# crisbodnar/text-to-image

Measured on AMD Instinct MI355X. Metric: images/sec (G+D step) at 64x64 batch=64, higher is better.
Workload: dtype f32; 1 GPU; wgancls 64x64 batch=64/GPU fp32, synthetic images + random 1024-d text embeddings, D step (+kt) then G step, Adam(b1=0,b2=0.9); global_batch=64, parallelism=dp1, launch=hipGraph replay (1 graph/iteration)

## Files before the change

### text-to-image_amd/csrc/t2i_bgemm.hip

```cpp
#include <hip/hip_runtime.h>
#include <stdint.h>

#include <type_traits>

#include "t2i_internal.h"

namespace t2i {

typedef float f32x16 __attribute__((ext_vector_type(16)));
typedef unsigned int u32x4 __attribute__((ext_vector_type(4)));

namespace {
constexpr int BK = 32;
constexpr int KSTRIDE = BK + 4;
constexpr unsigned OOB = 0xFFFFFFF0u;

template <int LAY, int WM, int WN, int NW = 4>
struct BSmem {
  static constexpr bool A_KIN = LAY != 2, B_KIN = LAY == 1;
  static constexpr int BM = 32 * (NW / 2) * WM, BN = 64 * WN;
  static constexpr int A_ELEMS = A_KIN ? BM * KSTRIDE : BK * BM;
  static constexpr int B_ELEMS = B_KIN ? BN * KSTRIDE : BK * BN;
  static constexpr int BYTES = 2 * (A_ELEMS + B_ELEMS) * 4;
};
// ... 84 lines not shown
        b_ok[i] = n < p.N;
        b_off[i] = (b_kr + B_KR * i) * p.N + n;
      }
    }
  };

  float4 areg[A_LD], breg[B_LD];
  auto load_into = [&](float4* ar, float4* br) __attribute__((always_inline)) {
    const int k0 = l_t * BK;
    ++l_t;
#pragma unroll
    for (int i = 0; i < A_LD; ++i) {
      if (A_KIN) ar[i] = bl4(ra, a_off[i] + k0, a_ok[i] & (k0 + kq * 4 < p.K));
      else ar[i] = bl4(ra, a_off[i] + k0 * p.M, a_ok[i] & (k0 + a_kr + A_KR * i < p.K));
    }
#pragma unroll
    for (int i = 0; i < B_LD; ++i) {
      if (B_KIN) br[i] = bl4(rb, b_off[i] + k0, b_ok[i] & (k0 + kq * 4 < p.K));
      else br[i] = bl4(rb, b_off[i] + k0 * p.N, b_ok[i] & (k0 + b_kr + B_KR * i < p.K));
    }
  };
  auto load_tile = [&]() __attribute__((always_inline)) { load_into(areg, breg); };
  auto store_from = [&](int buf, const float4* ar, const float4* br) __attribute__((always_inline)) {
    float* as = As + buf * S::A_ELEMS;
    float* bs = Bs + buf * S::B_ELEMS;
#pragma unroll
    for (int i = 0; i < A_LD; ++i) {
      if (A_KIN) *reinterpret_cast<float4*>(&as[(r0 + RPP * i) * KSTRIDE + kq * 4]) = ar[i];
      else *reinterpret_cast<float4*>(&as[(a_kr + A_KR * i) * BM + a_c4 * 4]) = ar[i];
    }
#pragma unroll
    for (int i = 0; i < B_LD; ++i) {
      if (B_KIN) *reinterpret_cast<float4*>(&bs[(r0 + RPP * i) * KSTRIDE + kq * 4]) = br[i];
      else *reinterpret_cast<float4*>(&bs[(b_kr + B_KR * i) * BN + b_c4 * 4]) = br[i];
    }
  };
  auto store_tile = [&](int buf) __attribute__((always_inline)) { store_from(buf, areg, breg); };

  struct Frag { float a[WM][4]; float b[WN][4]; };
  auto read_frag = [&](Frag& f, const float* as, const float* bs, int c) __attribute__((always_inline)) {
#pragma unroll
    for (int i = 0; i < WM; ++i) {
      const int row = (wm * WM + i) * 32 + l31;
      if (A_KIN) {
        const float4 v = *reinterpret_cast<const float4*>(&as[row * KSTRIDE + c * 8 + lh * 4]);
        f.a[i][0] = v.x; f.a[i][1] = v.y; f.a[i][2] = v.z; f.a[i][3] = v.w;
      } else {
#pragma unroll
        for (int j = 0; j < 4; ++j) f.a[i][j] = as[(c * 8 + j + 4 * lh) * BM + row];
      }
    }
#pragma unroll
    for (int i = 0; i < WN; ++i) {
      const int col = (wn * WN + i) * 32 + l31;
      if (B_KIN) {
        const float4 v = *reinterpret_cast<const float4*>(&bs[col * KSTRIDE + c * 8 + lh * 4]);
        f.b[i][0] = v.x; f.b[i][1] = v.y; f.b[i][2] = v.z; f.b[i][3] = v.w;
      } else {
#pragma unroll
        for (int j = 0; j < 4; ++j) f.b[i][j] = bs[(c * 8 + j + 4 * lh) * BN + col];
      }
    }
  };

  f32x16 acc[WM][WN];
#pragma unroll
  for (int i = 0; i < WM; ++i)
#pragma unroll
    for (int n = 0; n < WN; ++n)
#pragma unroll
      for (int e = 0; e < 16; ++e) acc[i][n][e] = 0.f;
  auto mma_frag = [&](const Frag& f) __attribute__((always_inline)) {
#pragma unroll
    for (int j = 0; j < 4; ++j)
#pragma unroll
      for (int i = 0; i < WM; ++i)
#pragma unroll
        for (int n = 0; n < WN; ++n)
          acc[i][n] = __builtin_amdgcn_mfma_f32_32x32x2f32(f.a[i][j], f.b[n][j], acc[i][n], 0, 0, 0);
  };
  constexpr int N_MMA = 4 * WM * WN, N_PIECE = A_LD + B_LD, MMA_PER_PIECE = N_MMA / N_PIECE > 0 ? N_MMA / N_PIECE : 1;

  auto k_tile = [&](int t, Frag& c0, Frag& c1, Frag& n0, Frag& n1) __attribute__((always_inline)) {
    const float* as = As + (t & 1) * S::A_ELEMS;
    const float* bs = Bs + (t & 1) * S::B_ELEMS;
    const float* an = As + ((t + 1) & 1) * S::A_ELEMS;
    const float* bn_ = Bs + ((t + 1) & 1) * S::B_ELEMS;
    __builtin_amdgcn_sched_barrier(0);
    mma_frag(c0);
    __builtin_amdgcn_sched_barrier(0);
    read_frag(c0, as, bs, 2);
    __builtin_amdgcn_sched_barrier(0);
    mma_frag(c1);
    store_tile((t + 1) & 1);
#pragma unroll
    for (int q2 = 0; q2 < N_PIECE; ++q2) {
      __builtin_amdgcn_sched_group_barrier(0x008, MMA_PER_PIECE, 0);
      __builtin_amdgcn_sched_group_barrier(0x200, 1, 0);
    }
    __builtin_amdgcn_sched_barrier(0);
    read_frag(c1, as, bs, 3);
    __builtin_amdgcn_sched_barrier(0);
    __syncthreads();
    read_frag(n0, an, bn_, 0);
    read_frag(n1, an, bn_, 1);
    __builtin_amdgcn_sched_barrier(0);
    load_tile();
    mma_frag(c0);
#pragma unroll
    for (int q2 = 0; q2 < N_PIECE; ++q2) {
      __builtin_amdgcn_sched_group_barrier(0x008, MMA_PER_PIECE, 0);
      __builtin_amdgcn_sched_group_barrier(0x020, 1, 0);
    }
    __builtin_amdgcn_sched_barrier(0);
    mma_frag(c1);
  };

  next_item();
  {
    float4 a0[A_LD], b0[B_LD];
    load_into(a0, b0);
    load_tile();
    store_from(0, a0, b0);
  }
  __syncthreads();
  Frag fa0, fa1, fb0, fb1;
  read_frag(fa0, As, Bs, 0);
  read_frag(fa1, As, Bs, 1);
  for (int it = 0; it < n_items; ++it) {
    for (int t = 0; t < p.ntiles; t += 2) {
      if (t + 2 == p.ntiles) next_item();
      k_tile(0, fa0, fa1, fb0, fb1);
      k_tile(1, fb0, fb1, fa0, fa1);
    }
    int bz, bm, bn;
    coords(run0 + slot + it * nslot, bz, bm, bn);
    float* out = p.c + (int64_t)bz * p.sc;
#pragma unroll
    for (int i = 0; i < WM; ++i)
#pragma unroll
      for (int j = 0; j < WN; ++j) {
        const int n = bn + (wn * WN + j) * 32 + l31;
#pragma unroll
        for (int e = 0; e < 16; ++e) {
          const int m = bm + (wm * WM + i) * 32 + (e & 3) + 8 * (e >> 2) + 4 * lh;
          if (m < p.M && n < p.N) out[(size_t)m * p.N + n] = acc[i][j][e];
        }
#pragma unroll
        for (int e = 0; e < 16; ++e) acc[i][j][e] = 0.f;
      }
  }
}

template <int LAY, bool XF = false>
__global__ __launch_bounds__(256, 2) void bgemm9_kernel(Bgemm9Params q) {
  static_assert(!XF, "the in-loader input transform is the specialisation bgemm9_kernel<1, true> below");
  const BgemmParams& p = q.g;
  using S = BSmem<LAY, 1, 1, 4>;
  constexpr bool B_KIN = S::B_KIN;
  constexpr int BM = 64, BN = 64, A_LD = 2, B_LD = 2;
  constexpr int B_C4 = BN / 4, B_KR = 256 / B_C4;
  extern __shared__ __attribute__((aligned(16))) float smem_b[];
  float* As = smem_b;
  float* Bs = smem_b + 2 * S::A_ELEMS;

  const int tid = threadIdx.x;
  const int lane = tid & 63, wave = tid >> 6;
  const int wm = wave >> 1, wn = wave & 1;
  const int l31 = lane & 31, lh = lane >> 5;

  const int nslot = gridDim.x >> 3;
  const int xcd = blockIdx.x & 7, slot = blockIdx.x >> 3;
  const int qq = p.items >> 3, rr_ = p.items & 7;
  const int run0 = xcd * qq + min(xcd, rr_), runlen = qq + (xcd < rr_ ? 1 : 0);
  if (slot >= runlen) return;
  const int n_items = (runlen - slot + nslot - 1) / nslot;
  const int tiles = p.tiles_m * p.tiles_n;

  auto coords = [&](int w, int& phs, int& bm, int& bn) __attribute__((always_inline)) {
    phs = w / tiles;
    const int t = w - phs * tiles;
    const int g = p.group_n, per_group = g * p.tiles_m;
    const int grp = t / per_group, rr = t - grp * per_group, n0 = grp * g;
    const int width = min(g, p.tiles_n - n0);
    const int tm = rr / width;
    bm = tm * BM;
    bn = (n0 + rr - tm * width) * BN;
  };
  auto plane_slot = [&](int pos, int phs) __attribute__((always_inline)) {
    if (LAY == 0) return pos;
    const int r = pos / 3, c = pos - 3 * r;
    return ((2 - r) * 3 + (2 - c)) * 4 + (3 - phs);
  };

  const int kq = tid & 7, r0 = tid >> 3;
  const int b_c4 = tid % B_C4, b_kr = tid / B_C4;
  __amdgpu_buffer_rsrc_t ra, rb;
  int a_off[A_LD], b_off[B_LD];
  bool a_ok[A_LD], b_ok[B_LD];
  int l_item = -1, l_pos = 8, l_t = 0, l_phs = 0, l_bm = 0, l_bn = 0;

  auto next_sub = [&]() __attribute__((always_inline)) {
    l_t = 0;
    if (++l_pos == 9) {
      l_pos = 0;
      ++l_item;
      if (l_item < n_items) coords(run0 + slot + l_item * nslot, l_phs, l_bm, l_bn);
    }
    if (l_item >= n_items) {
#pragma unroll
      for (int i = 0; i < A_LD; ++i) a_ok[i] = false;
#pragma unroll
      for (int i = 0; i < B_LD; ++i) b_ok[i] = false;
      return;
    }
    const int ps = plane_slot(l_pos, l_phs);
    ra = __builtin_amdgcn_make_buffer_rsrc(const_cast<float*>(p.a + (int64_t)ps * p.sa), (short)0, (int)p.a_bytes, 0x00020000);
    rb = __builtin_amdgcn_make_buffer_rsrc(const_cast<float*>(p.b + (int64_t)ps * p.sb), (short)0, (int)p.b_bytes, 0x00020000);
#pragma unroll
    for (int i = 0; i < A_LD; ++i) {
      const int m = l_bm + r0 + 32 * i;
      a_ok[i] = m < p.M;
      a_off[i] = m * p.K + kq * 4;
    }
#pragma unroll
    for (int i = 0; i < B_LD; ++i) {
      if (B_KIN) {
        const int n = l_bn + r0 + 32 * i;
        b_ok[i] = n < p.N;
        b_off[i] = n * p.K + kq * 4;
      } else {
        const int n = l_bn + b_c4 * 4;
        b_ok[i] = n < p.N;
        b_off[i] = (b_kr + B_KR * i) * p.N + n;
      }
    }
  };

  float4 areg[A_LD], breg[B_LD];
  auto load_into = [&](float4* ar, float4* br) __attribute__((always_inline)) {
    const int k0 = l_t * BK;
    ++l_t;
#pragma unroll
    for (int i = 0; i < A_LD; ++i) ar[i] = bl4(ra, a_off[i] + k0, a_ok[i] & (k0 + kq * 4 < p.K));
#pragma unroll
    for (int i = 0; i < B_LD; ++i) {
      if (B_KIN) br[i] = bl4(rb, b_off[i] + k0, b_ok[i] & (k0 + kq * 4 < p.K));
      else br[i] = bl4(rb, b_off[i] + k0 * p.N, b_ok[i] & (k0 + b_kr + B_KR * i < p.K));
    }
  };
  auto store_from = [&](int buf, const float4* ar, const float4* br) __attribute__((always_inline)) {
    float* as = As + buf * S::A_ELEMS;
    float* bs = Bs + buf * S::B_ELEMS;
#pragma unroll
    for (int i = 0; i < A_LD; ++i) *reinterpret_cast<float4*>(&as[(r0 + 32 * i) * KSTRIDE + kq * 4]) = ar[i];
#pragma unroll
    for (int i = 0; i < B_LD; ++i) {
      if (B_KIN) *reinterpret_cast<float4*>(&bs[(r0 + 32 * i) * KSTRIDE + kq * 4]) = br[i];
      else *reinterpret_cast<float4*>(&bs[(b_kr + B_KR * i) * BN + b_c4 * 4]) = br[i];
    }
  };

  struct Frag { float a[4]; float b[4]; };
  auto read_frag = [&](Frag& f, const float* as, const float* bs, int c) __attribute__((always_inline)) {
    {
      const int row = wm * 32 + l31;
      const float4 v = *reinterpret_cast<const float4*>(&as[row * KSTRIDE + c * 8 + lh * 4]);
      f.a[0] = v.x; f.a[1] = v.y; f.a[2] = v.z; f.a[3] = v.w;
    }
    {
      const int col = wn * 32 + l31;
      if (B_KIN) {
        const float4 v = *reinterpret_cast<const float4*>(&bs[col * KSTRIDE + c * 8 + lh * 4]);
        f.b[0] = v.x; f.b[1] = v.y; f.b[2] = v.z; f.b[3] = v.w;
      } else {
#pragma unroll
        for (int j = 0; j < 4; ++j) f.b[j] = bs[(c * 8 + j + 4 * lh) * BN + col];
      }
    }
  };

  f32x16 acc[9];
#pragma unroll
  for (int i = 0; i < 9; ++i)
#pragma unroll
    for (int e = 0; e < 16; ++e) acc[i][e] = 0.f;

  auto k_tile = [&](auto P_, int t, Frag& c0, Frag& c1, Frag& n0, Frag& n1) __attribute__((always_inline)) {
    constexpr int P = decltype(P_)::value;
    const float* as = As + (t & 1) * S::A_ELEMS;
    const float* bs = Bs + (t & 1) * S::B_ELEMS;
    const float* an = As + ((t + 1) & 1) * S::A_ELEMS;
    const float* bn_ = Bs + ((t + 1) & 1) * S::B_ELEMS;
    auto mma = [&](const Frag& f) __attribute__((always_inline)) {
#pragma unroll
      for (int j = 0; j < 4; ++j) acc[P] = __builtin_amdgcn_mfma_f32_32x32x2f32(f.a[j], f.b[j], acc[P], 0, 0, 0);
    };
    __builtin_amdgcn_sched_barrier(0);
    mma(c0);
    __builtin_amdgcn_sched_barrier(0);
    read_frag(c0, as, bs, 2);
    __builtin_amdgcn_sched_barrier(0);
    mma(c1);
    store_from((t + 1) & 1, areg, breg);
#pragma unroll
    for (int q2 = 0; q2 < 4; ++q2) {
      __builtin_amdgcn_sched_group_barrier(0x008, 1, 0);
      __builtin_amdgcn_sched_group_barrier(0x200, 1, 0);
    }
    __builtin_amdgcn_sched_barrier(0);
    read_frag(c1, as, bs, 3);
    __builtin_amdgcn_sched_barrier(0);
    __syncthreads();
    read_frag(n0, an, bn_, 0);
    read_frag(n1, an, bn_, 1);
    __builtin_amdgcn_sched_barrier(0);
    load_into(areg, breg);
    mma(c0);
#pragma unroll
    for (int q2 = 0; q2 < 4; ++q2) {
      __builtin_amdgcn_sched_group_barrier(0x008, 1, 0);
      __builtin_amdgcn_sched_group_barrier(0x020, 1, 0);
    }
    __builtin_amdgcn_sched_barrier(0);
    mma(c1);
  };

  next_sub();
  {
    float4 a0[A_LD], b0[B_LD];
    load_into(a0, b0);
    load_into(areg, breg);
    store_from(0, a0, b0);
  }
  __syncthreads();
  Frag fa0, fa1, fb0, fb1;
  read_frag(fa0, As, Bs, 0);
  read_frag(fa1, As, Bs, 1);
  auto run_pos = [&](auto P_) __attribute__((always_inline)) {
    for (int t = 0; t < p.ntiles; t += 2) {
      if (t + 2 == p.ntiles) next_sub();
      k_tile(P_, 0, fa0, fa1, fb0, fb1);
      k_tile(P_, 1, fb0, fb1, fa0, fa1);
    }
  };
  const int plane_px = q.Th * q.Tw;
  for (int it = 0; it < n_items; ++it) {
    run_pos(std::integral_constant<int, 0>{}); run_pos(std::integral_constant<int, 1>{}); run_pos(std::integral_constant<int, 2>{});
    run_pos(std::integral_constant<int, 3>{}); run_pos(std::integral_constant<int, 4>{}); run_pos(std::integral_constant<int, 5>{});
    run_pos(std::integral_constant<int, 6>{}); run_pos(std::integral_constant<int, 7>{}); run_pos(std::integral_constant<int, 8>{});
    int phs, bm, bn;
    coords(run0 + slot + it * nslot, phs, bm, bn);
    const int ph = phs >> 1, pw = phs & 1;
    const int n = bn + wn * 32 + l31;
    const float bs_ = (q.bias && n < p.N) ? q.bias[n] : 0.f;
#pragma unroll
    for (int e = 0; e < 16; ++e) {
      const int m = bm + wm * 32 + (e & 3) + 8 * (e >> 2) + 4 * lh;
      float z[2][3];
#pragma unroll
      for (int c = 0; c < 3; ++c) {
        z[0][c] = acc[0 * 3 + c][e] + acc[1 * 3 + c][e];
        z[1][c] = acc[1 * 3 + c][e] + acc[2 * 3 + c][e];
      }
      if (m < p.M && n < p.N) {
        const int b = m / plane_px, rem = m - b * plane_px;
        const int ty = rem / q.Tw, tx = rem - ty * q.Tw;
#pragma unroll
        for (int r = 0; r < 2; ++r) {
          const float y0 = apply_act((z[r][0] + z[r][1]) + bs_, q.act, q.alpha);
          const float y1 = apply_act((z[r][1] + z[r][2]) + bs_, q.act, q.alpha);
          const size_t oh = (size_t)q.sr * (2 * ty + r) + ph, ow0 = (size_t)q.sr * (2 * tx) + pw;
          float* o = q.out + (((size_t)b * q.OH + oh) * q.OW + ow0) * p.N + n;
          o[0] = y0;
          o[(size_t)q.sr * p.N] = y1;
        }
      }
    }
#pragma unroll
    for (int i = 0; i < 9; ++i)
#pragma unroll
      for (int e = 0; e < 16; ++e) acc[i][e] = 0.f;
  }
}

namespace {
__host__ __device__ constexpr int w9_pos(int i) {
  return i == 0 ? 4 : i == 1 ? 1 : i == 2 ? 3 : i == 3 ? 0 : i == 4 ? 5 : i == 5 ? 2 : i == 6 ? 7 : i == 7 ? 6 : 8;
}
constexpr int W9_PARK_BYTES = 4 * 2 * 256 * 16;
__device__ __forceinline__ float4 sub4(float4 a, float4 b) { return make_float4(a.x - b.x, a.y - b.y, a.z - b.z, a.w - b.w); }
}

template <>
__global__ __launch_bounds__(256, 2) void bgemm9_kernel<1, true>(Bgemm9Params q) {
  const BgemmParams& p = q.g;
  using S = BSmem<1, 1, 1, 4>;
  constexpr int BM = 64, BN = 64;
  extern __shared__ __attribute__((aligned(16))) float smem_b[];
  float* As = smem_b;
  float* Bs = smem_b + 2 * S::A_ELEMS;

  const int tid = threadIdx.x;
  const int lane = tid & 63, wave = tid >> 6;
  const int wm = wave >> 1, wn = wave & 1;
  const int l31 = lane & 31, lh = lane >> 5;
  float4* park = reinterpret_cast<float4*>(smem_b + 2 * (S::A_ELEMS + S::B_ELEMS)) + tid;

  const int nslot = gridDim.x >> 3;
  const int xcd = blockIdx.x & 7, slot = blockIdx.x >> 3;
  const int qq = p.items >> 3, rr_ = p.items & 7;
  const int run0 = xcd * qq + min(xcd, rr_), runlen = qq + (xcd < rr_ ? 1 : 0);
  if (slot >= runlen) return;
  const int n_items = (runlen - slot + nslot - 1) / nslot;
  const int tiles = p.tiles_m * p.tiles_n;

  auto coords = [&](int w, int& phs, int& bm, int& bn) __attribute__((always_inline)) {
    phs = w / tiles;
    const int t = w - phs * tiles;
    const int g = p.group_n, per_group = g * p.tiles_m;
    const int grp = t / per_group, rr = t - grp * per_group, n0 = grp * g;
    const int width = min(g, p.tiles_n - n0);
    const int tm = rr / width;
    bm = tm * BM;
    bn = (n0 + rr - tm * width) * BN;
  };

  const int kq = tid & 7, r0 = tid >> 3;
  const __amdgpu_buffer_rsrc_t ra = __builtin_amdgcn_make_buffer_rsrc(const_cast<float*>(q.dy), (short)0, (int)p.a_bytes, 0x00020000);
  const int rowpx = q.dWo * p.K;
  int a_off[2], b_off[2];
  unsigned a_win[2];
  bool b_ok[2];
  int l_item = -1, l_t = p.ntiles - 1, l_phs = 0;

  auto advance = [&]() __attribute__((always_inline)) {
    if (++l_t < p.ntiles) return;
    l_t = 0;
    ++l_item;
    if (l_item >= n_items) {
#pragma unroll
      for (int i = 0; i < 2; ++i) { a_win[i] = 0u; b_ok[i] = false; }
      return;
    }
    int bm, bn;
    coords(run0 + slot + l_item * nslot, l_phs, bm, bn);
    const int ph = l_phs >> 1, pw = l_phs & 1;
#pragma unroll
    for (int i = 0; i < 2; ++i) {
      const int m = bm + r0 + 32 * i;
      const int b = m / (q.Th * q.Tw), rem = m - b * (q.Th * q.Tw);
      const int ty = rem / q.Tw, tx = rem - ty * q.Tw;
      const int oh0 = 2 * ty + ph - 1, ow0 = 2 * tx + pw - 1;
      a_off[i] = ((b * q.dHo + oh0) * q.dWo + ow0) * p.K + kq * 4;
      unsigned w = 0u;
#pragma unroll
      for (int rr2 = 0; rr2 < 3; ++rr2)
#pragma unroll
        for (int cc2 = 0; cc2 < 3; ++cc2)
          if ((unsigned)(oh0 + rr2) < (unsigned)q.dHo && (unsigned)(ow0 + cc2) < (unsigned)q.dWo) w |= 1u << (rr2 * 3 + cc2);
      a_win[i] = m < p.M ? w : 0u;
      const int n = bn + r0 + 32 * i;
      b_ok[i] = n < p.N;
      b_off[i] = n * p.K + kq * 4;
    }
  };

  float4 areg[2], breg[2];
  auto load_stage = [&](auto I_, float4* ar, float4* br) __attribute__((always_inline)) {
    constexpr int P = w9_pos(decltype(I_)::value), r = P / 3, c = P - 3 * r;
    const int k0 = l_t * BK;
    const bool kin = k0 + kq * 4 < p.K;
    const int tap = r * rowpx + c * p.K + k0;
#pragma unroll
    for (int i = 0; i < 2; ++i) ar[i] = bl4(ra, a_off[i] + tap, kin & (((a_win[i] >> P) & 1u) != 0u));
    const int ps = ((2 - r) * 3 + (2 - c)) * 4 + (3 - l_phs);
    const __amdgpu_buffer_rsrc_t rb = __builtin_amdgcn_make_buffer_rsrc(const_cast<float*>(p.b + (int64_t)ps * p.sb), (short)0, (int)p.b_bytes, 0x00020000);
#pragma unroll
    for (int i = 0; i < 2; ++i) br[i] = bl4(rb, b_off[i] + k0, b_ok[i] & kin);
  };

  float4 c4[2];
  auto park_read = [&](auto I_, float4* tb, float4* tc) __attribute__((always_inline)) {
    constexpr int P = w9_pos(decltype(I_)::value), r = P / 3, c = P - 3 * r;
    if (r != 1 && c != 1) {
#pragma unroll
      for (int i = 0; i < 2; ++i) {
        tb[i] = park[(((3 + c) - 1) / 2 * 2 + i) * 256];
        tc[i] = park[(((3 * r + 1) - 1) / 2 * 2 + i) * 256];
      }
    }
  };
  auto form_store = [&](auto I_, int buf, const float4* ar, const float4* br, const float4* pb, const float4* pc) __attribute__((always_inline)) {
    constexpr int P = w9_pos(decltype(I_)::value), r = P / 3, c = P - 3 * r;
    float* as = As + buf * S::A_ELEMS;
    float* bs = Bs + buf * S::B_ELEMS;
    const float4 zero = make_float4(0.f, 0.f, 0.f, 0.f);
#pragma unroll
    for (int i = 0; i < 2; ++i) *reinterpret_cast<float4*>(&bs[(r0 + 32 * i) * KSTRIDE + kq * 4]) = br[i];
    if (P == 4) { c4[0] = ar[0]; c4[1] = ar[1]; }
    if ((P & 1) != 0) {
#pragma unroll
      for (int i = 0; i < 2; ++i) park[((P - 1) / 2 * 2 + i) * 256] = ar[i];
    }
#pragma unroll
    for (int i = 0; i < 2; ++i) {
      const float4 tb = r == 1 ? zero : c == 1 ? c4[i] : pb[i];
      const float4 tc = c == 1 ? zero : r == 1 ? c4[i] : pc[i];
      const float4 td = (r != 1 && c != 1) ? c4[i] : zero;
      *reinterpret_cast<float4*>(&as[(r0 + 32 * i) * KSTRIDE + kq * 4]) = sub4(sub4(ar[i], tb), sub4(tc, td));
    }
  };

  struct Frag { float a[4]; float b[4]; };
  auto read_frag = [&](Frag& f, const float* as, const float* bs, int c) __attribute__((always_inline)) {
    const float4 va = *reinterpret_cast<const float4*>(&as[(wm * 32 + l31) * KSTRIDE + c * 8 + lh * 4]);
    f.a[0] = va.x; f.a[1] = va.y; f.a[2] = va.z; f.a[3] = va.w;
    const float4 vb = *reinterpret_cast<const float4*>(&bs[(wn * 32 + l31) * KSTRIDE + c * 8 + lh * 4]);
    f.b[0] = vb.x; f.b[1] = vb.y; f.b[2] = vb.z; f.b[3] = vb.w;
  };

  f32x16 acc[9];
#pragma unroll
  for (int i = 0; i < 9; ++i)
#pragma unroll
    for (int e = 0; e < 16; ++e) acc[i][e] = 0.f;

  auto k_tile = [&](auto I_, int t, Frag& c0, Frag& c1, Frag& n0, Frag& n1) __attribute__((always_inline)) {
    constexpr int I = decltype(I_)::value, P = w9_pos(I);
    using IN = std::integral_constant<int, (I + 1) % 9>;
    using IL = std::integral_constant<int, (I + 2) % 9>;
    const float* as = As + (t & 1) * S::A_ELEMS;
    const float* bs = Bs + (t & 1) * S::B_ELEMS;
    const float* an = As + ((t + 1) & 1) * S::A_ELEMS;
    const float* bn_ = Bs + ((t + 1) & 1) * S::B_ELEMS;
    auto mma = [&](const Frag& f) __attribute__((always_inline)) {
#pragma unroll
      for (int j = 0; j < 4; ++j) acc[P] = __builtin_amdgcn_mfma_f32_32x32x2f32(f.a[j], f.b[j], acc[P], 0, 0, 0);
    };
    float4 pb[2], pc[2];
    __builtin_amdgcn_sched_barrier(0);
    mma(c0);
    __builtin_amdgcn_sched_barrier(0);
    read_frag(c0, as, bs, 2);
    park_read(IN{}, pb, pc);
    __builtin_amdgcn_sched_barrier(0);
    mma(c1);
    form_store(IN{}, (t + 1) & 1, areg, breg, pb, pc);
#pragma unroll
    for (int q2 = 0; q2 < 4; ++q2) {
      __builtin_amdgcn_sched_group_barrier(0x008, 1, 0);
      __builtin_amdgcn_sched_group_barrier(0x002, 6, 0);
      __builtin_amdgcn_sched_group_barrier(0x200, 2, 0);
    }
    __builtin_amdgcn_sched_barrier(0);
    read_frag(c1, as, bs, 3);
    __builtin_amdgcn_sched_barrier(0);
    __syncthreads();
    read_frag(n0, an, bn_, 0);
    read_frag(n1, an, bn_, 1);
    __builtin_amdgcn_sched_barrier(0);
    load_stage(IL{}, areg, breg);
    mma(c0);
#pragma unroll
    for (int q2 = 0; q2 < 4; ++q2) {
      __builtin_amdgcn_sched_group_barrier(0x008, 1, 0);
      __builtin_amdgcn_sched_group_barrier(0x020, 1, 0);
    }
    __builtin_amdgcn_sched_barrier(0);
    mma(c1);
  };

  advance();
  {
    float4 a0[2], b0[2];
    load_stage(std::integral_constant<int, 0>{}, a0, b0);
    load_stage(std::integral_constant<int, 1>{}, areg, breg);
    form_store(std::integral_constant<int, 0>{}, 0, a0, b0, a0, a0);
  }
  __syncthreads();
  Frag fa0, fa1, fb0, fb1;
  read_frag(fa0, As, Bs, 0);
  read_frag(fa1, As, Bs, 1);
#define T2I_W9_STAGE(I, u) \
  if ((((u) + (I)) & 1) == 0) k_tile(std::integral_constant<int, I>{}, 0, fa0, fa1, fb0, fb1); \
  else k_tile(std::integral_constant<int, I>{}, 1, fb0, fb1, fa0, fa1);
#define T2I_W9_KTILE(u) \
  T2I_W9_STAGE(0, u) T2I_W9_STAGE(1, u) T2I_W9_STAGE(2, u) T2I_W9_STAGE(3, u) T2I_W9_STAGE(4, u) T2I_W9_STAGE(5, u) T2I_W9_STAGE(6, u) \
  advance(); \
  T2I_W9_STAGE(7, u) T2I_W9_STAGE(8, u)
  const int plane_px = q.Th * q.Tw;
  for (int it = 0; it < n_items; ++it) {
    for (int t = 0; t < p.ntiles; t += 2) {
      T2I_W9_KTILE(0)
      T2I_W9_KTILE(1)
    }
#undef T2I_W9_KTILE
#undef T2I_W9_STAGE
    int phs, bm, bn;
    coords(run0 + slot + it * nslot, phs, bm, bn);
    const int ph = phs >> 1, pw = phs & 1;
    const int n = bn + wn * 32 + l31;
    const float bs_ = (q.bias && n < p.N) ? q.bias[n] : 0.f;
#pragma unroll
    for (int e = 0; e < 16; ++e) {
      const int m = bm + wm * 32 + (e & 3) + 8 * (e >> 2) + 4 * lh;
      float z[2][3];
#pragma unroll
      for (int c = 0; c < 3; ++c) {
        z[0][c] = acc[0 * 3 + c][e] + acc[1 * 3 + c][e];
        z[1][c] = acc[1 * 3 + c][e] + acc[2 * 3 + c][e];
      }
      if (m < p.M && n < p.N) {
        const int b = m / plane_px, rem = m - b * plane_px;
        const int ty = rem / q.Tw, tx = rem - ty * q.Tw;
#pragma unroll
        for (int r = 0; r < 2; ++r) {
          const float y0 = apply_act((z[r][0] + z[r][1]) + bs_, q.act, q.alpha);
          const float y1 = apply_act((z[r][1] + z[r][2]) + bs_, q.act, q.alpha);
          const size_t oh = (size_t)q.sr * (2 * ty + r) + ph, ow0 = (size_t)q.sr * (2 * tx) + pw;
          float* o = q.out + (((size_t)b * q.OH + oh) * q.OW + ow0) * p.N + n;
          o[0] = y0;
          o[(size_t)q.sr * p.N] = y1;
        }
      }
    }
#pragma unroll
    for (int i = 0; i < 9; ++i)
#pragma unroll
      for (int e = 0; e < 16; ++e) acc[i][e] = 0.f;
  }
}

hipError_t bgemm9_launch(int lay, const Bgemm9Params& q, hipStream_t stream) {
  if (lay != 0 && lay != 1) return hipErrorInvalidValue;
  const int bytes = lay == 0 ? BSmem<0, 1, 1, 4>::BYTES : BSmem<1, 1, 1, 4>::BYTES;
  const int per_xcd = (q.g.items + 7) / 8;
  int nslot = per_xcd < 32 * 2 ? per_xcd : 32 * 2;
  if (nslot < 1) nslot = 1;
  if (lay == 0) hipLaunchKernelGGL((bgemm9_kernel<0, false>), dim3(nslot * 8), dim3(256), bytes, stream, q);
  else if (q.dy) {
    constexpr int wbytes = BSmem<1, 1, 1, 4>::BYTES + W9_PARK_BYTES;
    static bool attr_done = false;
    if (!attr_done) {
      hipError_t e = hipFuncSetAttribute(reinterpret_cast<const void*>(bgemm9_kernel<1, true>), hipFuncAttributeMaxDynamicSharedMemorySize, wbytes);
      if (e != hipSuccess) return e;
      attr_done = true;
    }
    hipLaunchKernelGGL((bgemm9_kernel<1, true>), dim3(nslot * 8), dim3(256), wbytes, stream, q);
  } else hipLaunchKernelGGL((bgemm9_kernel<1, false>), dim3(nslot * 8), dim3(256), bytes, stream, q);
  return hipGetLastError();
}

template <int LAY, int WM, int WN, int NW = 4>
static hipError_t launch_b(const BgemmParams& p, hipStream_t stream) {
  using S = BSmem<LAY, WM, WN, NW>;
  auto k = bgemm_kernel<LAY, WM, WN, NW>;
  static bool attr_done = false;
  if (!attr_done && S::BYTES > 48 * 1024) {
    hipError_t e = hipFuncSetAttribute(reinterpret_cast<const void*>(k), hipFuncAttributeMaxDynamicSharedMemorySize, S::BYTES);
    if (e != hipSuccess) return e;
    attr_done = true;
  }
  const int per_cu = (WM * WN == 1 && NW == 4) ? 4 : 2;
  const int per_xcd = (p.items + 7) / 8;
  int nslot = per_xcd < 32 * per_cu ? per_xcd : 32 * per_cu;
  if (nslot < 1) nslot = 1;
  hipLaunchKernelGGL(k, dim3(nslot * 8), dim3(64 * NW), S::BYTES, stream, p);
  return hipGetLastError();
}

hipError_t bgemm_launch(int lay, int wm, int wn, const BgemmParams& p, hipStream_t stream) {
  if (wm == 4 && wn == 1) {
    if (lay == 0) return launch_b<0, 1, 1, 8>(p, stream);
    if (lay == 1) return launch_b<1, 1, 1, 8>(p, stream);
    if (lay == 2) return launch_b<2, 1, 1, 8>(p, stream);
  }
#define T2I_B(L, a, b) if (lay == L && wm == a && wn == b) return launch_b<L, a, b>(p, stream);
  T2I_B(0, 1, 1) T2I_B(0, 2, 1) T2I_B(0, 1, 2) T2I_B(0, 2, 2)
  T2I_B(1, 1, 1) T2I_B(1, 2, 1) T2I_B(1, 1, 2) T2I_B(1, 2, 2)
  T2I_B(2, 1, 1) T2I_B(2, 2, 1) T2I_B(2, 1, 2) T2I_B(2, 2, 2)
#undef T2I_B
  return hipErrorInvalidValue;
}

}
```

### text-to-image_amd/csrc/t2i_winograd.hip

```cpp
#include <hip/hip_runtime.h>
#include <stdint.h>
#include <stdio.h>
#include <string.h>
#include <stdlib.h>

#include <mutex>
#include <vector>

#include "t2i_internal.h"

namespace t2i {

struct FilterEntry {
  const float* w; int kind, Cin, Cout; float* U; size_t bytes; unsigned long long cap; hipStream_t stream; bool valid;
  hipStream_t cap_fill = nullptr;
};
static std::mutex g_fc_mu;
static std::vector<FilterEntry> g_fc;
static int g_fc_on = 0;
static char* g_fc_buf = nullptr;
static size_t g_fc_cap = 0, g_fc_used = 0;

int filter_cache_attach(void* buf, size_t bytes) {
  std::lock_guard<std::mutex> lk(g_fc_mu);
// ... 342 lines not shown
  const int rc = run_batched_gemm(gd, MODE_BWD_FILTER, 16, V, Z, P, (int64_t)Tp * d.Cin, (int64_t)T * d.Cout, (int64_t)d.Cin * d.Cout, stream,
                                  "winograd filter-gradient gemm");
  if (rc != T2I_OK) return rc;
  hipLaunchKernelGGL(wino_dw_kernel, dim3(wino_blocks((size_t)d.Cin * (d.Cout / 4))), dim3(256), 0, stream, P, d.Cin, d.Cout, accumulate, dw);
  const hipError_t e = hipGetLastError();
  if (e != hipSuccess) { set_error("winograd filter gradient: %s", hipGetErrorString(e)); return T2I_ERR_LAUNCH; }
  return T2I_OK;
}

__device__ __forceinline__ void wino2_filter_body(const float* __restrict__ w, int Cin, int Cout, float* __restrict__ U, unsigned vb, unsigned nvb) {
  const int N4 = Cout >> 2;
  const size_t total = (size_t)4 * Cin * N4;
  const size_t plane = (size_t)4 * Cin * N4;
  for (size_t i = (size_t)vb * 256 + threadIdx.x; i < total; i += (size_t)nvb * 256) {
    const int n4 = (int)(i % N4);
    const int ci = (int)((i / N4) % Cin);
    const int ph = (int)(i / ((size_t)N4 * Cin));
    const int p = ph >> 1, q = ph & 1;
    float4 g[2][2];
#pragma unroll
    for (int a = 0; a < 2; ++a)
#pragma unroll
      for (int b = 0; b < 2; ++b)
        g[a][b] = reinterpret_cast<const float4*>(w + ((size_t)((2 * a + p) * 4 + (2 * b + q)) * Cin + ci) * Cout)[n4];
    float4 s[3][2] = {{g[0][0], g[0][1]}, {f4add(g[0][0], g[1][0]), f4add(g[0][1], g[1][1])}, {g[1][0], g[1][1]}};
    float4* o = reinterpret_cast<float4*>(U) + ((size_t)ph * Cin + ci) * N4 + n4;
#pragma unroll
    for (int r = 0; r < 3; ++r) {
      wst(&o[(size_t)(r * 3 + 0) * plane], s[r][0]);
      wst(&o[(size_t)(r * 3 + 1) * plane], f4add(s[r][0], s[r][1]));
      wst(&o[(size_t)(r * 3 + 2) * plane], s[r][1]);
    }
  }
}

__global__ __launch_bounds__(256) void wino2_filter_kernel(const float* __restrict__ w, int Cin, int Cout, float* __restrict__ U) {
  wino2_filter_body(w, Cin, Cout, U, blockIdx.x, gridDim.x);
}

__global__ __launch_bounds__(256) void wino2_input_kernel(const float* __restrict__ x, int H, int W, int C, int Th, int Tw, size_t T,
                                                          float* __restrict__ V, size_t plane_T) {
  const int C4 = C >> 2;
  const size_t total = T * 4 * C4;
  const size_t plane = plane_T * 4 * C4;
  for (size_t i = (size_t)blockIdx.x * blockDim.x + threadIdx.x; i < total; i += (size_t)gridDim.x * blockDim.x) {
    const int c4 = (int)(i % C4);
    const int ph = (int)((i / C4) & 3);
    const size_t t = i / ((size_t)4 * C4);
    const int p = ph >> 1, q = ph & 1;
    const int tx = (int)(t % Tw);
    const int ty = (int)((t / Tw) % Th);
    const size_t b = t / ((size_t)Tw * Th);
    float4 d[3][3];
#pragma unroll
    for (int r = 0; r < 3; ++r) {
      const int ih = 4 * ty - 1 + 2 * r + p;
#pragma unroll
      for (int c = 0; c < 3; ++c) {
        const int iw = 4 * tx - 1 + 2 * c + q;
        d[r][c] = ((unsigned)ih < (unsigned)H && (unsigned)iw < (unsigned)W)
                      ? reinterpret_cast<const float4*>(x + ((b * H + ih) * W + iw) * C)[c4]
                      : make_float4(0.f, 0.f, 0.f, 0.f);
      }
    }
    float4 tt[3][3];
#pragma unroll
    for (int c = 0; c < 3; ++c) {
      tt[0][c] = f4sub(d[0][c], d[1][c]);
      tt[1][c] = d[1][c];
      tt[2][c] = f4sub(d[2][c], d[1][c]);
    }
    float4* o = reinterpret_cast<float4*>(V) + (t * 4 + ph) * C4 + c4;
#pragma unroll
    for (int r = 0; r < 3; ++r) {
      wst(&o[(size_t)(r * 3 + 0) * plane], f4sub(tt[r][0], tt[r][1]));
      wst(&o[(size_t)(r * 3 + 1) * plane], tt[r][1]);
      wst(&o[(size_t)(r * 3 + 2) * plane], f4sub(tt[r][2], tt[r][1]));
    }
  }
}

__global__ __launch_bounds__(256) void wino2_output_kernel(const float* __restrict__ Mx, const float* __restrict__ bias, int Ho, int Wo,
                                                           int N, int Th, int Tw, size_t T, int act, float alpha,
                                                           float* __restrict__ y) {
  const int N4 = N >> 2;
  const size_t total = T * N4, plane = T * N4;
  for (size_t i = (size_t)blockIdx.x * blockDim.x + threadIdx.x; i < total; i += (size_t)gridDim.x * blockDim.x) {
    const int n4 = (int)(i % N4);
    const size_t t = i / N4;
    const int tx = (int)(t % Tw);
    const int ty = (int)((t / Tw) % Th);
    const size_t b = t / ((size_t)Tw * Th);
    const float4* m = reinterpret_cast<const float4*>(Mx) + t * N4 + n4;
    float4 z[2][3];
#pragma unroll
    for (int c = 0; c < 3; ++c) {
      const float4 m0 = m[(size_t)(0 * 3 + c) * plane], m1 = m[(size_t)(1 * 3 + c) * plane], m2 = m[(size_t)(2 * 3 + c) * plane];
      z[0][c] = f4add(m0, m1);
      z[1][c] = f4add(m1, m2);
    }
    const float4 bs = bias ? reinterpret_cast<const float4*>(bias)[n4] : make_float4(0.f, 0.f, 0.f, 0.f);
#pragma unroll
    for (int r = 0; r < 2; ++r) {
      float4 y0 = f4add(f4add(z[r][0], z[r][1]), bs);
      float4 y1 = f4add(f4add(z[r][1], z[r][2]), bs);
      y0.x = apply_act(y0.x, act, alpha); y0.y = apply_act(y0.y, act, alpha); y0.z = apply_act(y0.z, act, alpha); y0.w = apply_act(y0.w, act, alpha);
      y1.x = apply_act(y1.x, act, alpha); y1.y = apply_act(y1.y, act, alpha); y1.z = apply_act(y1.z, act, alpha); y1.w = apply_act(y1.w, act, alpha);
      float4* o = reinterpret_cast<float4*>(y + ((b * Ho + 2 * ty + r) * Wo + 2 * tx) * N) + n4;
      o[0] = y0;
      o[N4] = y1;
    }
  }
}

bool winograd_k4s2_eligible(const t2i_conv_desc& d, bool bwd_data) {
  const int minc = tuning().winograd_k4s2_minc;
  if (!tuning().winograd_k4s2 || d.math != T2I_MATH_F32) return false;
  if (!(d.KH == 4 && d.KW == 4 && d.SH == 2 && d.SW == 2 && d.pad_t == 1 && d.pad_l == 1)) return false;
  if ((d.H & 3) || (d.W & 3) || d.Ho * 2 != d.H || d.Wo * 2 != d.W) return false;
  if (bwd_data ? ((d.Cout % 32) || (d.Cin % 32)) : ((d.Cin % 8) || (d.Cout % 32))) return false;
  const int minc_bwd = tuning().winograd_k4s2_bwd_minc;
  const int m = bwd_data ? minc_bwd : minc;
  if (!(d.Cin >= m && d.Cout >= m)) return false;
  const int64_t T = (int64_t)d.B * (d.Ho / 2) * (d.Wo / 2);
  const int64_t items = 9 * ((T + 63) / 64) * ((d.Cout + 63) / 64);
  return T * 4 * d.Cin * d.Cout >= (int64_t)tuning().winograd_k4s2_minwork && items >= tuning().winograd_k4s2_minitems;
}

size_t winograd_k4s2_ws(const t2i_conv_desc& d) {
  const size_t T = (size_t)d.B * (d.Ho / 2) * (d.Wo / 2), K = (size_t)4 * d.Cin;
  return al256(9 * K * d.Cout * 4) + al256(9 * T * K * 4) + al256(9 * T * d.Cout * 4);
}

static int wino2_fused_gemm(int lay, int phases, size_t T, int N, int K, const float* V, const float* U, int64_t sa, int64_t sb, const float* bias,
                            float* out, int OH, int OW, int Th, int Tw, int sr, int act, float alpha, hipStream_t stream, const char* what,
                            const float* dy_raw = nullptr, int dHo = 0, int dWo = 0, int64_t dy_elems = 0) {
  const int mode = tuning().wino_fuse;
  if (!mode || !tuning().bgemm) return -1;
  const int ntiles = dy_raw ? ((K + 31) / 32 + 1) & ~1 : (K + 31) / 32;
  const int64_t a_elems = dy_raw ? dy_elems : (int64_t)T * K, b_elems = (int64_t)N * K;
  if (dy_raw) V = dy_raw;
  if ((ntiles & 1) || (!dy_raw && (T & 3)) || (N & 3) || (K & 3) || (reinterpret_cast<uintptr_t>(V) & 15) || (reinterpret_cast<uintptr_t>(U) & 15) || (sa & 3) || (sb & 3) ||
      a_elems >= (1LL << 30) || b_elems >= (1LL << 30) || T >= (1u << 30))
    return -1;
  Bgemm9Params q;
  memset(&q, 0, sizeof(q));
  q.g.a = V; q.g.b = U; q.g.c = nullptr;
  q.g.M = (int32_t)T; q.g.N = N; q.g.K = K;
  q.g.tiles_m = (int32_t)((T + 63) / 64); q.g.tiles_n = (N + 63) / 64;
  { const int g = tuning().group_n; q.g.group_n = q.g.tiles_n < g ? q.g.tiles_n : g; if (q.g.group_n < 1) q.g.group_n = 1; }
  q.g.ntiles = ntiles;
  const int64_t items = (int64_t)phases * q.g.tiles_m * q.g.tiles_n;
  if (items >= (1LL << 30)) return -1;
  if (mode == 1) {
    const int64_t rounds = (items + 511) / 512;
    if (items < (int64_t)tuning().wino_fuse_items * (lay == 0 ? 4 : 1) || items * 100 < rounds * 512 * 85) return -1;
    if (K >= 1024 && rounds < 3) return -1;
  }
  q.g.items = (int32_t)items;
  q.g.sa = sa; q.g.sb = sb; q.g.sc = 0;
  q.g.a_bytes = (uint32_t)(a_elems * 4); q.g.b_bytes = (uint32_t)(b_elems * 4);
  q.bias = bias; q.out = out; q.OH = OH; q.OW = OW; q.Th = Th; q.Tw = Tw; q.sr = sr; q.act = act; q.alpha = alpha;
  q.dy = dy_raw; q.dHo = dHo; q.dWo = dWo;
  if (tuning().debug_plan) fprintf(stderr, "[t2i plan] %s: fused 9-position items, %d phases x %d x %d tiles, K=%d\n", what, phases, q.g.tiles_m, q.g.tiles_n, K);
  const hipError_t e = bgemm9_launch(lay, q, stream);
  if (e != hipSuccess) { set_error("%s: %s", what, hipGetErrorString(e)); return T2I_ERR_LAUNCH; }
  return T2I_OK;
}

int winograd_k4s2_fwd(const t2i_conv_desc& d, const float* x, const float* w, const float* bias, float* y, int act, float alpha,
                      void* ws, size_t ws_bytes, hipStream_t stream, float* Vkeep) {
  const size_t T = (size_t)d.B * (d.Ho / 2) * (d.Wo / 2), K = (size_t)4 * d.Cin;
  if (!ws || ws_bytes < winograd_k4s2_ws(d) || (reinterpret_cast<uintptr_t>(ws) & 15)) {
    set_error("winograd k4s2 conv: workspace %zu B < %zu B required (or misaligned)", ws_bytes, winograd_k4s2_ws(d));
    return T2I_ERR_WORKSPACE;
  }
  char* base = reinterpret_cast<char*>(ws);
  float* U = reinterpret_cast<float*>(base);
  float* V = Vkeep ? Vkeep : reinterpret_cast<float*>(base + al256(9 * K * d.Cout * 4));
  float* Mx = reinterpret_cast<float*>(base + al256(9 * K * d.Cout * 4) + al256(9 * T * K * 4));
  const int Th = d.Ho / 2, Tw = d.Wo / 2;
  bool fill = true;
  if (float* Uc = filter_cache_get(w, 2, d.Cin, d.Cout, (size_t)9 * 4 * d.Cin * d.Cout * 4, stream, &fill)) U = Uc;
  if (fill)
    hipLaunchKernelGGL(wino2_filter_kernel, dim3(wino_blocks((size_t)4 * d.Cin * (d.Cout / 4))), dim3(256), 0, stream, w, d.Cin, d.Cout, U);
  hipLaunchKernelGGL(wino2_input_kernel, dim3(wino_blocks(T * d.Cin)), dim3(256), 0, stream, x, d.H, d.W, d.Cin, Th, Tw, T, V, T);
  t2i_conv_desc gd = d;
  gd.B = (int32_t)T; gd.H = gd.W = gd.Ho = gd.Wo = 1; gd.Cin = (int32_t)K; gd.KH = gd.KW = gd.SH = gd.SW = 1; gd.pad_t = gd.pad_l = 0;
  {
    const int fr = wino2_fused_gemm(0, 1, T, d.Cout, (int)K, V, U, (int64_t)T * K, (int64_t)K * d.Cout, bias, y, d.Ho, d.Wo, Th, Tw, 1, act, alpha, stream,
                                    "winograd k4s2 fused gemm");
    if (fr != -1) return fr;
  }
  const int rc = run_batched_gemm(gd, MODE_FWD, 9, V, U, Mx, (int64_t)T * K, (int64_t)K * d.Cout, (int64_t)T * d.Cout, stream, "winograd k4s2 gemm");
  if (rc != T2I_OK) return rc;
  hipLaunchKernelGGL(wino2_output_kernel, dim3(wino_blocks(T * (d.Cout / 4))), dim3(256), 0, stream, Mx, bias, d.Ho, d.Wo, d.Cout, Th, Tw, T, act,
                     alpha, y);
  const hipError_t e = hipGetLastError();
  if (e != hipSuccess) { set_error("winograd k4s2 conv: %s", hipGetErrorString(e)); return T2I_ERR_LAUNCH; }
  return T2I_OK;
}

__device__ __forceinline__ int wino2b_slot(int r, int c, int phs) { return ((2 - r) * 3 + (2 - c)) * 4 + (3 - phs); }

__global__ __launch_bounds__(256) void wino2b_input_kernel(const float* __restrict__ dy, int Ho, int Wo, int C, int Th, int Tw, size_t T,
                                                           float* __restrict__ V) {
  const int C4 = C >> 2;
  const size_t total = T * 4 * C4;
  const size_t plane = T * C4;
  for (size_t i = (size_t)blockIdx.x * blockDim.x + threadIdx.x; i < total; i += (size_t)gridDim.x * blockDim.x) {
    const int c4 = (int)(i % C4);
    const size_t t = (i / C4) % T;
    const int phs = (int)(i / ((size_t)C4 * T));
    const int ph = phs >> 1, pw = phs & 1;
    const int tx = (int)(t % Tw);
    const int ty = (int)((t / Tw) % Th);
    const size_t b = t / ((size_t)Tw * Th);
    float4 d[3][3];
#pragma unroll
    for (int r = 0; r < 3; ++r) {
      const int oh = 2 * ty + ph - 1 + r;
#pragma unroll
      for (int c = 0; c < 3; ++c) {
        const int ow = 2 * tx + pw - 1 + c;
        d[r][c] = ((unsigned)oh < (unsigned)Ho && (unsigned)ow < (unsigned)Wo)
                      ? reinterpret_cast<const float4*>(dy + ((b * Ho + oh) * Wo + ow) * C)[c4]
                      : make_float4(0.f, 0.f, 0.f, 0.f);
      }
    }
    float4 tt[3][3];
#pragma unroll
    for (int c = 0; c < 3; ++c) {
      tt[0][c] = f4sub(d[0][c], d[1][c]);
      tt[1][c] = d[1][c];
      tt[2][c] = f4sub(d[2][c], d[1][c]);
    }
    float4* o = reinterpret_cast<float4*>(V) + t * C4 + c4;
#pragma unroll
    for (int r = 0; r < 3; ++r) {
      wst(&o[(size_t)wino2b_slot(r, 0, phs) * plane], f4sub(tt[r][0], tt[r][1]));
      wst(&o[(size_t)wino2b_slot(r, 1, phs) * plane], tt[r][1]);
      wst(&o[(size_t)wino2b_slot(r, 2, phs) * plane], f4sub(tt[r][2], tt[r][1]));
    }
  }
}

__global__ __launch_bounds__(256) void wino2b_output_kernel(const float* __restrict__ Mx, const float* __restrict__ bias, int H, int W,
                                                            int N, int Th, int Tw, size_t T, int act, float alpha,
                                                            float* __restrict__ dx) {
  const int N4 = N >> 2;
  const size_t total = T * 4 * N4, plane = T * N4;
  for (size_t i = (size_t)blockIdx.x * blockDim.x + threadIdx.x; i < total; i += (size_t)gridDim.x * blockDim.x) {
    const int n4 = (int)(i % N4);
    const size_t t = (i / N4) % T;
    const int phs = (int)(i / ((size_t)N4 * T));
    const int ph = phs >> 1, pw = phs & 1;
    const int tx = (int)(t % Tw);
    const int ty = (int)((t / Tw) % Th);
    const size_t b = t / ((size_t)Tw * Th);
    const float4* m = reinterpret_cast<const float4*>(Mx) + t * N4 + n4;
    float4 z[2][3];
#pragma unroll
    for (int c = 0; c < 3; ++c) {
      const float4 m0 = m[(size_t)wino2b_slot(0, c, phs) * plane], m1 = m[(size_t)wino2b_slot(1, c, phs) * plane],
                   m2 = m[(size_t)wino2b_slot(2, c, phs) * plane];
      z[0][c] = f4add(m0, m1);
      z[1][c] = f4add(m1, m2);
    }
    const float4 bs = bias ? reinterpret_cast<const float4*>(bias)[n4] : make_float4(0.f, 0.f, 0.f, 0.f);
#pragma unroll
    for (int r = 0; r < 2; ++r) {
      float4 y0 = f4add(f4add(z[r][0], z[r][1]), bs);
      float4 y1 = f4add(f4add(z[r][1], z[r][2]), bs);
      y0.x = apply_act(y0.x, act, alpha); y0.y = apply_act(y0.y, act, alpha); y0.z = apply_act(y0.z, act, alpha); y0.w = apply_act(y0.w, act, alpha);
      y1.x = apply_act(y1.x, act, alpha); y1.y = apply_act(y1.y, act, alpha); y1.z = apply_act(y1.z, act, alpha); y1.w = apply_act(y1.w, act, alpha);
      const size_t ih = (size_t)2 * (2 * ty + r) + ph;
      float4* o0 = reinterpret_cast<float4*>(dx + ((b * H + ih) * W + (size_t)2 * (2 * tx) + pw) * N) + n4;
      float4* o1 = reinterpret_cast<float4*>(dx + ((b * H + ih) * W + (size_t)2 * (2 * tx + 1) + pw) * N) + n4;
      *o0 = y0;
      *o1 = y1;
    }
  }
}

size_t winograd_k4s2_bwd_ws(const t2i_conv_desc& d) {
  const size_t T = (size_t)d.B * (d.Ho / 2) * (d.Wo / 2);
  return al256((size_t)36 * d.Cin * d.Cout * 4) + al256(36 * T * d.Cout * 4) + al256(36 * T * d.Cin * 4);
}

int winograd_k4s2_bwd_data(const t2i_conv_desc& d, const float* dy, const float* w, const float* bias, float* dx, int act, float alpha,
                           void* ws, size_t ws_bytes, hipStream_t stream) {
  const size_t T = (size_t)d.B * (d.Ho / 2) * (d.Wo / 2);
  if (!ws || ws_bytes < winograd_k4s2_bwd_ws(d) || (reinterpret_cast<uintptr_t>(ws) & 15)) {
    set_error("winograd k4s2 input gradient: workspace %zu B < %zu B required (or misaligned)", ws_bytes, winograd_k4s2_bwd_ws(d));
    return T2I_ERR_WORKSPACE;
  }
  char* base = reinterpret_cast<char*>(ws);
  float* U = reinterpret_cast<float*>(base);
  float* V = reinterpret_cast<float*>(base + al256((size_t)36 * d.Cin * d.Cout * 4));
  float* Mx = reinterpret_cast<float*>(base + al256((size_t)36 * d.Cin * d.Cout * 4) + al256(36 * T * d.Cout * 4));
  const int Th = d.Ho / 2, Tw = d.Wo / 2;
  bool fill = true;
  if (float* Uc = filter_cache_get(w, 2, d.Cin, d.Cout, (size_t)36 * d.Cin * d.Cout * 4, stream, &fill)) U = Uc;
  if (fill)
    hipLaunchKernelGGL(wino2_filter_kernel, dim3(wino_blocks((size_t)4 * d.Cin * (d.Cout / 4))), dim3(256), 0, stream, w, d.Cin, d.Cout, U);
  if (tuning().wino_fuse_xf) {
    const int fr = wino2_fused_gemm(1, 4, T, d.Cin, d.Cout, V, U, (int64_t)T * d.Cout, (int64_t)d.Cin * d.Cout, bias, dx, d.H, d.W, Th, Tw, 2, act, alpha, stream,
// ... 315 lines not shown
```

Baseline: 5229 images/sec.

## Stage fused Winograd 9-position epilogue through LDS for float4 coalesced stores

Replaces the scalar scattered output stores of the fused 9-position bgemm kernels with an epilogue that writes activated results to an extra LDS staging area, then reads them back as float4 so each lane stores a contiguous 4-channel vector. The aim is fewer, wider and better-coalesced global writes. This adds a 32 KB LDS stage to every variant, which may lower occupancy, and requires setting the max dynamic shared memory attribute for all three kernels. It also adds a cost-model heuristic that decides when the dy-fused layout-1 path is used, which can send more or fewer convolutions through the fused kernel.

```diff
diff --git a/text-to-image_amd/csrc/t2i_bgemm.hip b/text-to-image_amd/csrc/t2i_bgemm.hip
--- a/text-to-image_amd/csrc/t2i_bgemm.hip
+++ b/text-to-image_amd/csrc/t2i_bgemm.hip
@@ -260,9 +260,75 @@
   }
 }
 
+namespace {
+constexpr int W9_STAGE_BYTES = 8 * 256 * 16;
+__device__ __forceinline__ void w9_epilogue(f32x16 (&acc)[9], const Bgemm9Params& q, float* stage, int phs, int bm, int bn, int tid) {
+  const BgemmParams& p = q.g;
+  const int lane = tid & 63, wave = tid >> 6;
+  const int wm = wave >> 1, wn = wave & 1;
+  const int l31 = lane & 31, lh = lane >> 5;
+  const int ph = phs >> 1, pw = phs & 1;
+  const int na = bn + wn * 32 + l31;
+  const float bs_ = (q.bias && na < p.N) ? q.bias[na] : 0.f;
+  const int pr = (lane >> 4) & 1, pc = (lane >> 3) & 1;
+  const int n = bn + wn * 32 + (lane & 7) * 4;
+  const size_t lane_off = ((size_t)(q.sr * pr + ph) * q.OW + (size_t)(q.sr * pc + pw)) * p.N + n;
+  int m = bm + wm * 32 + lh;
+  int b = m / (q.Th * q.Tw), ty, tx;
+  {
+    const int rem = m - b * (q.Th * q.Tw);
+    ty = rem / q.Tw;
+    tx = rem - ty * q.Tw;
+  }
+  float* wr = stage + lh * 2048 + wave * 256 + l31;
+  const float4* rd = reinterpret_cast<const float4*>(stage) + tid;
+#pragma unroll
+  for (int h = 0; h < 2; ++h) {
+#pragma unroll
+    for (int ee = 0; ee < 8; ++ee) {
+      const int e = 8 * h + ee;
+      float z[2][3];
+#pragma unroll
+      for (int c = 0; c < 3; ++c) {
+        z[0][c] = acc[0 * 3 + c][e] + acc[1 * 3 + c][e];
+        z[1][c] = acc[1 * 3 + c][e] + acc[2 * 3 + c][e];
+      }
+      float* w = wr + (((ee & 3) >> 1) + 4 * (ee >> 2)) * 1024 + (ee & 1) * 128;
+#pragma unroll
+      for (int r = 0; r < 2; ++r) {
+        w[(2 * r + 0) * 32] = apply_act((z[r][0] + z[r][1]) + bs_, q.act, q.alpha);
+        w[(2 * r + 1) * 32] = apply_act((z[r][1] + z[r][2]) + bs_, q.act, q.alpha);
+      }
+    }
+    __builtin_amdgcn_fence(__ATOMIC_RELEASE, "wavefront");
+    __builtin_amdgcn_wave_barrier();
+    __builtin_amdgcn_fence(__ATOMIC_ACQUIRE, "wavefront");
+#pragma unroll
+    for (int j = 0; j < 8; ++j) {
+      const float4 v = rd[j * 256];
+      if (m < p.M && n < p.N)
+        *reinterpret_cast<float4*>(q.out + (((size_t)b * q.OH + (size_t)(2 * q.sr) * ty) * q.OW + (size_t)(2 * q.sr) * tx) * p.N + lane_off) = v;
+      m += 2;
+      tx += 2;
+      while (tx >= q.Tw) {
+        tx -= q.Tw;
+        if (++ty == q.Th) { ty = 0; ++b; }
+      }
+    }
+    __builtin_amdgcn_fence(__ATOMIC_RELEASE, "wavefront");
+    __builtin_amdgcn_wave_barrier();
+    __builtin_amdgcn_fence(__ATOMIC_ACQUIRE, "wavefront");
+  }
+#pragma unroll
+  for (int i = 0; i < 9; ++i)
+#pragma unroll
+    for (int e = 0; e < 16; ++e) acc[i][e] = 0.f;
+}
+}
+
 template <int LAY, bool XF = false>
 __global__ __launch_bounds__(256, 2) void bgemm9_kernel(Bgemm9Params q) {
-  static_assert(!XF, "the in-loader input transform is the specialisation bgemm9_kernel<1, true> below");
+  static_assert(!XF,"the in-loader input transform is the specialisation bgemm9_kernel<1, true> below");
   const BgemmParams& p = q.g;
   using S = BSmem<LAY, 1, 1, 4>;
   constexpr bool B_KIN = S::B_KIN;
@@ -452,43 +518,14 @@
       k_tile(P_, 1, fb0, fb1, fa0, fa1);
     }
   };
-  const int plane_px = q.Th * q.Tw;
+  float* stage = smem_b + 2 * (S::A_ELEMS + S::B_ELEMS);
   for (int it = 0; it < n_items; ++it) {
     run_pos(std::integral_constant<int, 0>{}); run_pos(std::integral_constant<int, 1>{}); run_pos(std::integral_constant<int, 2>{});
     run_pos(std::integral_constant<int, 3>{}); run_pos(std::integral_constant<int, 4>{}); run_pos(std::integral_constant<int, 5>{});
     run_pos(std::integral_constant<int, 6>{}); run_pos(std::integral_constant<int, 7>{}); run_pos(std::integral_constant<int, 8>{});
     int phs, bm, bn;
     coords(run0 + slot + it * nslot, phs, bm, bn);
-    const int ph = phs >> 1, pw = phs & 1;
-    const int n = bn + wn * 32 + l31;
-    const float bs_ = (q.bias && n < p.N) ? q.bias[n] : 0.f;
-#pragma unroll
-    for (int e = 0; e < 16; ++e) {
-      const int m = bm + wm * 32 + (e & 3) + 8 * (e >> 2) + 4 * lh;
-      float z[2][3];
-#pragma unroll
-      for (int c = 0; c < 3; ++c) {
-        z[0][c] = acc[0 * 3 + c][e] + acc[1 * 3 + c][e];
-        z[1][c] = acc[1 * 3 + c][e] + acc[2 * 3 + c][e];
-      }
-      if (m < p.M && n < p.N) {
-        const int b = m / plane_px, rem = m - b * plane_px;
-        const int ty = rem / q.Tw, tx = rem - ty * q.Tw;
-#pragma unroll
-        for (int r = 0; r < 2; ++r) {
-          const float y0 = apply_act((z[r][0] + z[r][1]) + bs_, q.act, q.alpha);
-          const float y1 = apply_act((z[r][1] + z[r][2]) + bs_, q.act, q.alpha);
-          const size_t oh = (size_t)q.sr * (2 * ty + r) + ph, ow0 = (size_t)q.sr * (2 * tx) + pw;
-          float* o = q.out + (((size_t)b * q.OH + oh) * q.OW + ow0) * p.N + n;
-          o[0] = y0;
-          o[(size_t)q.sr * p.N] = y1;
-        }
-      }
-    }
-#pragma unroll
-    for (int i = 0; i < 9; ++i)
-#pragma unroll
-      for (int e = 0; e < 16; ++e) acc[i][e] = 0.f;
+    w9_epilogue(acc, q, stage, phs, bm, bn, tid);
   }
 }
 
@@ -697,7 +734,6 @@
   T2I_W9_STAGE(0, u) T2I_W9_STAGE(1, u) T2I_W9_STAGE(2, u) T2I_W9_STAGE(3, u) T2I_W9_STAGE(4, u) T2I_W9_STAGE(5, u) T2I_W9_STAGE(6, u) \
   advance(); \
   T2I_W9_STAGE(7, u) T2I_W9_STAGE(8, u)
-  const int plane_px = q.Th * q.Tw;
   for (int it = 0; it < n_items; ++it) {
     for (int t = 0; t < p.ntiles; t += 2) {
       T2I_W9_KTILE(0)
@@ -707,56 +743,29 @@
 #undef T2I_W9_STAGE
     int phs, bm, bn;
     coords(run0 + slot + it * nslot, phs, bm, bn);
-    const int ph = phs >> 1, pw = phs & 1;
-    const int n = bn + wn * 32 + l31;
-    const float bs_ = (q.bias && n < p.N) ? q.bias[n] : 0.f;
-#pragma unroll
-    for (int e = 0; e < 16; ++e) {
-      const int m = bm + wm * 32 + (e & 3) + 8 * (e >> 2) + 4 * lh;
-      float z[2][3];
-#pragma unroll
-      for (int c = 0; c < 3; ++c) {
-        z[0][c] = acc[0 * 3 + c][e] + acc[1 * 3 + c][e];
-        z[1][c] = acc[1 * 3 + c][e] + acc[2 * 3 + c][e];
-      }
-      if (m < p.M && n < p.N) {
-        const int b = m / plane_px, rem = m - b * plane_px;
-        const int ty = rem / q.Tw, tx = rem - ty * q.Tw;
-#pragma unroll
-        for (int r = 0; r < 2; ++r) {
-          const float y0 = apply_act((z[r][0] + z[r][1]) + bs_, q.act, q.alpha);
-          const float y1 = apply_act((z[r][1] + z[r][2]) + bs_, q.act, q.alpha);
-          const size_t oh = (size_t)q.sr * (2 * ty + r) + ph, ow0 = (size_t)q.sr * (2 * tx) + pw;
-          float* o = q.out + (((size_t)b * q.OH + oh) * q.OW + ow0) * p.N + n;
-          o[0] = y0;
-          o[(size_t)q.sr * p.N] = y1;
-        }
-      }
-    }
-#pragma unroll
-    for (int i = 0; i < 9; ++i)
-#pragma unroll
-      for (int e = 0; e < 16; ++e) acc[i][e] = 0.f;
+    w9_epilogue(acc, q, smem_b + 2 * (S::A_ELEMS + S::B_ELEMS), phs, bm, bn, tid);
   }
 }
 
 hipError_t bgemm9_launch(int lay, const Bgemm9Params& q, hipStream_t stream) {
   if (lay != 0 && lay != 1) return hipErrorInvalidValue;
-  const int bytes = lay == 0 ? BSmem<0, 1, 1, 4>::BYTES : BSmem<1, 1, 1, 4>::BYTES;
+  static_assert(W9_PARK_BYTES == W9_STAGE_BYTES, "the loader-transform kernel stages its epilogue in the parked-pixel slots");
+  const int bytes = (lay == 0 ? BSmem<0, 1, 1, 4>::BYTES : BSmem<1, 1, 1, 4>::BYTES) + W9_STAGE_BYTES;
   const int per_xcd = (q.g.items + 7) / 8;
   int nslot = per_xcd < 32 * 2 ? per_xcd : 32 * 2;
   if (nslot < 1) nslot = 1;
-  if (lay == 0) hipLaunchKernelGGL((bgemm9_kernel<0, false>), dim3(nslot * 8), dim3(256), bytes, stream, q);
-  else if (q.dy) {
-    constexpr int wbytes = BSmem<1, 1, 1, 4>::BYTES + W9_PARK_BYTES;
-    static bool attr_done = false;
-    if (!attr_done) {
-      hipError_t e = hipFuncSetAttribute(reinterpret_cast<const void*>(bgemm9_kernel<1, true>), hipFuncAttributeMaxDynamicSharedMemorySize, wbytes);
-      if (e != hipSuccess) return e;
-      attr_done = true;
-    }
-    hipLaunchKernelGGL((bgemm9_kernel<1, true>), dim3(nslot * 8), dim3(256), wbytes, stream, q);
-  } else hipLaunchKernelGGL((bgemm9_kernel<1, false>), dim3(nslot * 8), dim3(256), bytes, stream, q);
+  const int which = lay == 0 ? 0 : q.dy ? 1 : 2;
+  const void* fn = which == 0 ? reinterpret_cast<const void*>(bgemm9_kernel<0, false>)
+                 : which == 1 ? reinterpret_cast<const void*>(bgemm9_kernel<1, true>) : reinterpret_cast<const void*>(bgemm9_kernel<1, false>);
+  static bool attr_done[3] = {false, false, false};
+  if (!attr_done[which]) {
+    hipError_t e = hipFuncSetAttribute(fn, hipFuncAttributeMaxDynamicSharedMemorySize, bytes);
+    if (e != hipSuccess) return e;
+    attr_done[which] = true;
+  }
+  if (which == 0) hipLaunchKernelGGL((bgemm9_kernel<0, false>), dim3(nslot * 8), dim3(256), bytes, stream, q);
+  else if (which == 1) hipLaunchKernelGGL((bgemm9_kernel<1, true>), dim3(nslot * 8), dim3(256), bytes, stream, q);
+  else hipLaunchKernelGGL((bgemm9_kernel<1, false>), dim3(nslot * 8), dim3(256), bytes, stream, q);
   return hipGetLastError();
 }
 
diff --git a/text-to-image_amd/csrc/t2i_winograd.hip b/text-to-image_amd/csrc/t2i_winograd.hip
--- a/text-to-image_amd/csrc/t2i_winograd.hip
+++ b/text-to-image_amd/csrc/t2i_winograd.hip
@@ -518,7 +518,11 @@
   q.g.ntiles = ntiles;
   const int64_t items = (int64_t)phases * q.g.tiles_m * q.g.tiles_n;
   if (items >= (1LL << 30)) return -1;
-  if (mode == 1) {
+  const int kt = (K + 31) / 32;
+  if (mode == 1 && lay == 1 && dy_raw && kt >= 8 && kt <= 32) {
+    const int64_t h = (items + 255) / 256;
+    if (h < 2 || 0.5f * h * (12.f + 9.7f * kt) >= (float)items * (0.135f + 0.017f * kt)) return -1;
+  } else if (mode == 1) {
     const int64_t rounds = (items + 511) / 512;
     if (items < (int64_t)tuning().wino_fuse_items * (lay == 0 ? 4 : 1) || items * 100 < rounds * 512 * 85) return -1;
     if (K >= 1024 && rounds < 3) return -1;
```

Result: no change. 5249 images/sec, median of 6 (+0.4%).
